# istellartech/OpenGoddard

Hardware: AMD Instinct MI355X
Metric: NLP-callback evals/sec (cost+constr+FD-Jacobian) (higher is better)
Workload: dtype f64; 1 GPU; polar_tsto: 2 phases, [6, 6] states, [3, 3] controls, [80, 80] LGL nodes; n=1442, m_eq=975, m_ineq=640, output_buffers=17 registered persistent-zero replicas of 18.6 MB in rotation, parallelism=fd-columns x1

## Files before the change

### __graft_entry__.py

```python
import os
import subprocess
import sys

ROOT = os.path.dirname(os.path.abspath(__file__))
if ROOT not in sys.path:
    sys.path.insert(0, ROOT)

PREBUILT = ("brachistochrone", "goddard", "polar_tsto_shipped", "polar_tsto",
            "low_thrust_shipped", "low_thrust", "launch4", "table_ascent", "low_thrust_r1", "launch4_r1",
            "goddard_1knot", "polar_ssto")


BEYOND_8192_NODES = [208, 208, 208, 208]
BOTH_CORES_NODES = [30]
NEAR_THE_LIMIT_NODES = [341, 341, 341, 341]


def build():
    from opengoddard_amd import build as ogbuild
    from opengoddard_amd import _native, codegen, problems
    print("[build] libogpsx.so ->", ogbuild.build_core(), flush=True)
    _native.lib()
    print("[build] libogsqp.so ->", ogbuild.build_sqp(), flush=True)
    from opengoddard_amd import _sqp_native
# ... 17 lines not shown
        import test_random_layouts
        extra = [factory() for factory in test_edge_problems.CASES.values()]
        extra += [test_random_layouts.make_problem(shape, seed) for seed, shape in test_random_layouts.CASES]
        for i, (prob, obj) in enumerate(extra):
            headers.append(("test problem %d" % i, codegen.emit_header(codegen.trace_problem(prob, obj))))
        import test_module_limits
        for key in test_module_limits.SHAPES:
            prob, obj = test_module_limits.problem(key)
            headers.append(("limit shape " + key, codegen.emit_header(codegen.trace_problem(prob, obj))))
            if key in test_module_limits.NOT_FITTING:
                batched.append(headers[-1])
        import test_fused_no_barrier
        for key in sorted(test_fused_no_barrier.SHAPES):
            prob, obj = test_fused_no_barrier.problem(key)
            headers.append(("no-barrier shape " + key, codegen.emit_header(codegen.trace_problem(prob, obj))))
        import test_exact_surface
        for name in test_exact_surface.BATCHED:
            prob, obj = test_exact_surface.build_problem(name)
            batched.append(("surface " + name, codegen.emit_header(codegen.trace_problem(prob, obj))))
        import warnings
        import parameter_cases
        for label, factory, with_batch in parameter_cases.modules():
            prob, obj = factory()
            with warnings.catch_warnings():
                warnings.simplefilter("ignore", RuntimeWarning)
                headers.append((label, codegen.emit_header(codegen.trace_problem(prob, obj))))
            if with_batch:
                batched.append(headers[-1])
                parametered.append(headers[-1])
        import og_math_cases
# ... 177 lines not shown
```

### opengoddard_amd/csrc/ogk.h

```cpp
#pragma once
#include <stdint.h>

#define OGK_ABI 14
#define OGK_MAX_PHASE 32

static inline int ogk_frag_nt(int N) { return (N + 15) / 16; }
static inline int ogk_frag_ks(int N) { return (N + 3) / 4; }
static inline long ogk_frag_size(int N) { return (long)ogk_frag_nt(N) * ogk_frag_ks(N) * 64; }
static inline void ogk_frag_pack(int N, const double* D, double* frag) {
    const int NT = ogk_frag_nt(N), KS = ogk_frag_ks(N);
    for (int nt = 0; nt < NT; ++nt)
        for (int ks = 0; ks < KS; ++ks)
            for (int lane = 0; lane < 64; ++lane) {
                const int k = 16 * nt + (lane & 15), l = 4 * ks + (lane >> 4);
                frag[((long)nt * KS + ks) * 64 + lane] = (k < N && l < N) ? D[(long)k * N + l] : 0.0;
            }
}

#define OGK_OTHER_PART (-4242)

enum ogk_mode {
    OGK_EVAL = 0,
    OGK_SWEEP = 1,
    OGK_DENSE = 2,
// ... 45 lines not shown
#define OGK_PART_HVP 9
#define OGK_PART_MIX 10
#define OGK_PART_HESS 11

enum ogk_flag {
    OGK_FLAG_COUNT_A = 0,
    OGK_FLAG_COUNT_B = 1,
    OGK_FLAG_TICKET = 2,
    OGK_FLAG_FUSED_COUNT = 3,
    OGK_FLAG_FUSED_RESULT = 4,
    OGK_FLAG_WORDS = 8
};

#ifdef __cplusplus
static_assert(OGK_FUSED == 5 && OGK_SWEEP == 1 && OGK_DENSE == 2, "og_sweep_mode's values are public (include/ogpsx.h)");
#endif

typedef struct ogk_info {
    int32_t abi;
    int32_t n, m, m_eq, m_ineq;
    int32_t n_phase, n_mv, n_groups, n_cvec;
    int32_t n_y0;
    int32_t phase_nodes[OGK_MAX_PHASE];
    int32_t n_eval_blocks;
    int32_t fused_ok;
} ogk_info;

typedef struct ogk_par_info {
    int32_t n_par, par_off;
} ogk_par_info;
// ... 5 lines not shown
    const double* cvec;
    double* f0;
    double* y0;
    double* xop;
    double* t0;
    double* z;
    int* nonfinite;
    int* nonfinite_next;
    unsigned* ready;
    double* jt;
    int32_t jt_sparse;
    int32_t jt_bump;
    uint32_t* jt_launches;
    uint32_t* jt_state;
    int* nonfinite_result;
    int32_t col_lo, col_hi;
    const int64_t* poff;
    const int64_t* pind;
    const int32_t* prow;
    int32_t* pint;
    double* pvals;
    double* ptail;
    int32_t ulo, uhi;
    double* trace;
    int64_t dfrag_off[OGK_MAX_PHASE];
} ogk_args;

#define OGK_BATCH_SETS 3
typedef struct ogk_batch_args {
    ogk_args* lanes;
// ... 22 lines not shown
```

### opengoddard_amd/csrc/ogk_fused_workgroup.inc

```
    int id = (int)blockIdx.x;
    if (id < n_eval) {
        FZ_TRACE_DECL(0);
        if (!(OGK_FZ & 16)) {
            if (id < ndef) eval_defect_body<true>(a, id, lds);
            else eval_rows_body<true>(a, id - ndef, lds);
        }
        FZ_STAMP(1);
        finish_eval(a, (unsigned)n_eval, reinterpret_cast<unsigned*>(lds));
        FZ_STAMP(4);
        FZ_TRACE_OUT(a);
        return;
    }
    id -= n_eval;
#ifndef OGK_ORDER
#define OGK_ORDER 0
#endif
    const int n_tile = OGT_N_FTILES, n_heavy = OGT_N_HPART;
    int kind, idx;
    if (OGK_ORDER == 0) {
        if (id < n_light) kind = 0, idx = id;
        else if (id < n_light + n_heavy) kind = 1, idx = id - n_light;
        else kind = 2, idx = id - n_light - n_heavy;
    } else if (OGK_ORDER == 1) {
        if (id < n_tile) kind = 2, idx = id;
        else if (id < n_tile + n_heavy) kind = 1, idx = id - n_tile;
        else kind = 0, idx = id - n_tile - n_heavy;
    } else {
        if (id < n_heavy) kind = 1, idx = id;
        else {
            const int r = id - n_heavy, pairs = n_light < n_tile ? n_light : n_tile;
            if (r < 2 * pairs) kind = (r & 1) ? 0 : 2, idx = r >> 1;
            else if (n_light > n_tile) kind = 0, idx = r - pairs;
            else kind = 2, idx = r - pairs;
        }
    }
    if (kind == 0)
        fz_light_body(a, n_sum < 0 ? group_lo + idx
                                   : idx < n_sum ? OGT_LSUM[sum_lo + idx] : OGT_LPLAIN[group_lo - sum_lo + idx - n_sum], lds);
    else if (kind == 1) { if (!(OGK_FZ & 32)) fz_heavy_part(a, idx, lds); }
    else fz_tile_body(a, idx, lds);
```

### opengoddard_amd/csrc/ogk_kernels.hip

```cpp
#include <hip/hip_runtime.h>
#include "ogk.h"
#include "og_dual.h"
#if defined(OGK_PART) && (OGK_PART == OGK_PART_HVP || OGK_PART == OGK_PART_MIX || OGK_PART == OGK_PART_HESS)
#include "og_dual2.h"
#endif
#include OG_GEN_HEADER

typedef double v4f64 __attribute__((ext_vector_type(4)));

#ifndef OGK_EXP
#define OGK_EXP 0
#endif

#ifndef OGK_TRACE
#define OGK_TRACE 0
#endif

namespace {

struct XCol {
    typedef double scalar;
    const double* x0;
    int j;
    double xj;
// ... 368 lines not shown
            const ogdual op = OgGen::mv_operand(si, l, xd, a.cvec);
            for (int k = tid; k < N; k += 256) {
                double v = __builtin_fma(op.d, dfrag_entry(a, phase, N, k, l), 0.0);
                if ((reads & 2) || ((reads & 1) && k == l)) v = v - OgGen::tail_one(si, k, xd, a.cvec).d;
                jrow[row0 + k] = v;
            }
        }
    }
}
#endif

constexpr int SWEEP_THREADS = 512;
constexpr int SWEEP_WAVES = SWEEP_THREADS / 64;

template <bool FUSED>
__device__ __forceinline__ void publish_row(const ogk_args& a, const int row, const double val) {
    const double zz = val - val;
    a.f0[row] = val;
    if (FUSED) __hip_atomic_store(&a.z[row], zz, __ATOMIC_RELAXED, __HIP_MEMORY_SCOPE_AGENT);
    else a.z[row] = zz;
    if (zz != zz) atomicAdd(a.nonfinite, 1);
}

template <bool FUSED>
__device__ __forceinline__ void eval_defect_body(const ogk_args& a, const int bx, double* lds) {
    const int4 blk = OGT_EVALBLK[bx];
    const int nt = blk.y, mv0 = blk.z, nmv = blk.w;
    const ogt_int8 rec0 = OGT_SLOT[mv0];
    const int N = rec0.v[0];
    const int KS = (N + 3) >> 2;
    const int NP = KS * 4;
    const int tid = (int)threadIdx.x;
    const int wave = tid >> 6, lane = tid & 63, lk = lane >> 4;

    double* dpanel = lds;
    double* xt = lds + KS * 64;
    double* ybuf = xt + OgGen::MAX_NMV * NP;
    const double* src = a.dfrag + a.dfrag_off[rec0.v[5]] + (long)nt * KS * 64;
    constexpr int UNR = 4;
// ... 52 lines not shown
    double T[TR];
#pragma unroll
    for (int r = 0; r < TR; ++r) {
        const int s = wave + r * SWEEP_WAVES;
        T[r] = (node_on && s < nmv) ? OgGen::tail_one(mv0 + s, k, base, a.cvec) : 0.0;
    }
    __syncthreads();
    if (!node_on) return;
#pragma unroll
    for (int r = 0; r < TR; ++r) {
        const int s = wave + r * SWEEP_WAVES;
        if (s >= nmv) break;
        const ogt_int8 rec = OGT_SLOT[mv0 + s];
        const double y = ybuf[s * 16 + lane];
        const int row = rec.v[3] + k;
        publish_row<FUSED>(a, row, y - T[r]);
        a.t0[row] = T[r];
        a.y0[rec.v[4] + k] = y;
    }
}

template <bool FUSED>
__device__ __forceinline__ void eval_rows_body(const ogk_args& a, const int bx, double* lds) {
    bool terms = false;
    if (TERM_CACHE) {
#pragma unroll
        for (int u = 0; u < SWEEP_WAVES; ++u) {
            const int w2 = bx * SWEEP_WAVES + u;
            if (w2 < OGT_N_ROWWAVES) terms = terms || OGT_ROWWAVE[w2].w != 0;
        }
        if (terms) {
            fill_terms<SWEEP_THREADS>(a, lds);
            __syncthreads();
        }
    }
    const int w = bx * SWEEP_WAVES + ((int)threadIdx.x >> 6);
    if (w >= OGT_N_ROWWAVES) return;
    const int4 rw = OGT_ROWWAVE[w];
    const int k = rw.y + ((int)threadIdx.x & 63);
    if (k >= rw.z) return;
    const XColT base = make_xcolt(a, -1, 0.0, terms ? lds : nullptr);
    int row;
    const double v = OgGen::item_value(rw.x, 0, k, base, a.y0, a.cvec, &row);
    publish_row<FUSED>(a, row, v);
}

#ifdef OGK_HAS_MAIN
__global__ __launch_bounds__(SWEEP_THREADS) void ogk_eval(const ogk_args a, const int ndef) {
    extern __shared__ __attribute__((aligned(16))) double lds[];
    const int id = (int)blockIdx.x;
    if (id == 0 && threadIdx.x == 0) {
        *a.nonfinite_next = 0;
        if (a.jt_bump) __hip_atomic_store(a.jt_launches, *a.jt_launches + 1u, __ATOMIC_RELAXED, __HIP_MEMORY_SCOPE_AGENT);
    }
    if (id < ndef) eval_defect_body<false>(a, id, lds);
    else eval_rows_body<false>(a, id - ndef, lds);
}
#endif

#ifndef OGK_LIGHT_COLS
#define OGK_LIGHT_COLS 4
#endif
constexpr int LIGHT_COLS = OGK_LIGHT_COLS;
constexpr int HEAVY_FLAG = 1 << 30;

__device__ __forceinline__ bool marked(const unsigned* bits, const int r) {
    return (bits[r >> 5] >> (r & 31)) & 1u;
}

__device__ __forceinline__ void fill_row(const ogk_args& a, double* jrow, const unsigned* bits,
                                         const int own_lo, const int own_hi, const int first,
// ... 254 lines not shown
    }
#endif
}

#ifndef OGK_FZ
#define OGK_FZ 0
#endif


__device__ __forceinline__ void lds_barrier() {
    __builtin_amdgcn_fence(__ATOMIC_RELEASE, "workgroup", "local");
    __builtin_amdgcn_s_barrier();
    __builtin_amdgcn_fence(__ATOMIC_ACQUIRE, "workgroup", "local");
}

__device__ __forceinline__ void fz_fill_from_z(const ogk_args& a, unsigned* bits) {
    const int tid = (int)threadIdx.x;
    for (int j = a.col_lo; j < a.col_hi; ++j) {
        const int4 col = OGT_COL[j];
        const int own_lo = col.z, own_hi = col.w & ~HEAVY_FLAG;
        for (int w = tid; w < ROW_WORDS; w += SWEEP_THREADS) bits[w] = 0u;
        __syncthreads();
        for (int e = col.x + tid; e < col.y; e += SWEEP_THREADS) {
            const int r = OGT_ELEM[e].w;
            atomicOr(&bits[r >> 5], 1u << (r & 31));
        }
        __syncthreads();
        fill_row(a, a.jt + (long)(j - a.col_lo) * OgGen::M, bits, own_lo, own_hi, tid, SWEEP_THREADS, false, true);
        __syncthreads();
    }
}

__device__ __forceinline__ void finish_eval(const ogk_args& a, const unsigned n_eval, unsigned* bits) {
    __shared__ int s_last;
    __builtin_amdgcn_s_waitcnt(0);
    __syncthreads();
    if (threadIdx.x == 0) {
        const unsigned t = __hip_atomic_fetch_add(a.ready, 1u, __ATOMIC_RELAXED, __HIP_MEMORY_SCOPE_AGENT);
        int last = 0;
        if (t + 1u == n_eval) {
            const int bad = __hip_atomic_load(a.nonfinite, __ATOMIC_RELAXED, __HIP_MEMORY_SCOPE_AGENT);
            const unsigned st = __hip_atomic_load(a.jt_state, __ATOMIC_RELAXED, __HIP_MEMORY_SCOPE_AGENT);
            const unsigned gen = __hip_atomic_load(a.jt_launches, __ATOMIC_RELAXED, __HIP_MEMORY_SCOPE_AGENT) + 1u;
            __hip_atomic_store(a.ready, 0u, __ATOMIC_RELAXED, __HIP_MEMORY_SCOPE_AGENT);
            __hip_atomic_store(a.jt_launches, gen, __ATOMIC_RELAXED, __HIP_MEMORY_SCOPE_AGENT);
            __hip_atomic_store(a.nonfinite_result, bad, __ATOMIC_RELAXED, __HIP_MEMORY_SCOPE_AGENT);
            if (a.ptail) a.ptail[OgGen::M] = (double)bad;
            __hip_atomic_store(a.nonfinite, 0, __ATOMIC_RELAXED, __HIP_MEMORY_SCOPE_AGENT);
            if (bad != 0) __hip_atomic_store(a.jt_state, gen, __ATOMIC_RELAXED, __HIP_MEMORY_SCOPE_AGENT);
            last = (bad != 0 || st == gen - 1u) ? 1 : 0;
        }
        s_last = last;
    }
    __syncthreads();
    if (s_last) fz_fill_from_z(a, bits);
}

template <int CH>
__device__ __forceinline__ void fz_load_panel(const double* bsrc, const int ks0, const int KS, double (&bv)[CH]) {
#pragma unroll
    for (int u = 0; u < CH; ++u) {
        const int ks = ks0 + u;
        const double v = bsrc[(ks < KS ? ks : KS - 1) * 64];
        bv[u] = ks < KS ? v : 0.0;
    }
}

template <int CH>
__device__ __forceinline__ void fz_load_first(const double* bsrc, const int KS, double (&b0)[CH], double (&b1)[CH]) {
    fz_load_panel<CH>(bsrc, 0, KS, b0);
// ... 281 lines not shown
            for (int r = 0; r < FZ_ROUNDS; ++r) {
                const double v = tyo[r] >= 0 ? t.yb[tyo[r] - y0_first] - tv[r] : tv[r];
                const double v0 = __shfl_down(v, 32);
                if (!base_role && il < cnt[r]) {
                    const double q = (v - v0) / dx;
                    jrow[trow[r]] = q;
                    if (pcol) pcol[tpos[r]] = q;
                }
            }
        }
    }
    FZ_STAMP(4);
    FZ_TRACE_OUT(a);
}

__device__ __forceinline__ void fz_tile_body(const ogk_args& a, const int bx, double* lds) {
    __shared__ int s_flags[4];
    FZ_TRACE_DECL(3);
    fz_sync_reset(s_flags, 4);
    const int4 tile = OGT_FTILE[bx];
    const int slot = tile.x, ct0 = tile.y, nt = tile.z, nct = tile.w;
    const ogt_int8 rec = OGT_SLOT[slot];
    const int N = rec.v[0], leaf = rec.v[2], row0 = rec.v[3];
    const bool diag = rec.v[6] & 1, generic = rec.v[6] & 2;
    const int dep0 = rec.v[7] >> 12, ndep = rec.v[7] & 0xfff;
    const int KS = (N + 3) >> 2;
    const int tid = (int)threadIdx.x;
    const int wave = tid >> 6, lane = tid & 63, lk = lane >> 4, kk = lane & 15;
    double* xt = lds;
    double* yb = lds + FZ_NP;
    double* tb = yb + 16;
// ... 37 lines not shown
        const XCol xa{a.x0, leaf + la, xa_b + xa_h};
        hit_v = OgGen::mv_operand(slot, la, xa, a.cvec);
    }
    if (col_on || wave == prod_wave) lds_count_wait(&s_flags[3], n_stage);
    FZ_STAMP(1);
    if (!col_wave) {
        if (wave == diag_wave) {
            if (diag_here && lk == 0 && k_on && leaf + k >= a.col_lo && leaf + k < a.col_hi) {
                const int jd = leaf + k;
                const double xbd = a.x0[jd];
                const XCol xd{a.x0, jd, xbd + a.h[jd]};
                td[kk] = OgGen::tail_one(slot, k, xd, a.cvec);
            }
            if (lane == 0) lds_count_up(&s_flags[2]);
        }
        if (wave == term_wave && lk == 0) tb[kk] = k_on ? OgGen::tail_one(slot, k, xbase, a.cvec) : 0.0;
        if (wave == term_wave && lane == 0) lds_count_up(&s_flags[1]);
        if (wave == prod_wave) {
            const v4f64 accb = fz_chain<CH>(bsrc, KS, b0, b1, [&](const int ks) {
                const double v = xt[(ks < KS ? ks : 0) * 4 + lk];
                return ks < KS ? v : 0.0;
            });
            if (lk == 0) yb[kk] = accb[0];
            FZ_STAMP(2);
            if (lane == 0) lds_count_up(&s_flags[0]);
        }
        FZ_TRACE_OUT(a);
        return;
    }
    if (!col_on) return;
    const int row = row0 + (k_on ? k : 0);
    double t_diag = 0.0;
    bool have_diag = false;
    {
        const int lc = k;
        const int reg = (lc - l0 - lk) >> 2;
        have_diag = diag && k_on && lc >= l0 + lk && ((lc - l0 - lk) & 3) == 0 && reg < 4 && lc < N &&
                    leaf + lc >= a.col_lo && leaf + lc < a.col_hi;
        if (have_diag && diag_wave < 0) {
            const int jd = leaf + lc;
// ... 39 lines not shown
            }
        }
        const double val = acc[reg] - t;
        const double q = (val - f_base) / dx;
        a.jt[(long)(j - a.col_lo) * OgGen::M + row] = q;
        if (a.pvals) a.pvals[a.poff[j] + k] = q;
    }
    FZ_STAMP(4);
    FZ_TRACE_OUT(a);
}

#ifndef OGK_FUSED_ATTR
#define OGK_FUSED_ATTR __attribute__((amdgpu_waves_per_eu(4)))
#endif
#ifdef OGK_HAS_FUSED
__global__ __launch_bounds__(SWEEP_THREADS) OGK_FUSED_ATTR void ogk_fused(const ogk_args a, const int ndef, const int n_eval,
                                                           const int group_lo, const int n_light, const int sum_lo,
                                                           const int n_sum) {
    extern __shared__ __attribute__((aligned(16))) double lds[];
#include "ogk_fused_workgroup.inc"
}
#endif

#if defined(OGK_HAS_BATCH) || defined(OGK_HAS_BATCH_EXACT) || defined(OGK_HAS_PAR) || defined(OGK_HAS_DIR) || \
    defined(OGK_HAS_ADJ) || defined(OGK_HAS_HVP) || defined(OGK_HAS_MIX) || defined(OGK_HAS_HESS)
typedef const ogk_args __attribute__((address_space(4))) * ogk_lane_table;
__device__ __forceinline__ const ogk_args& batch_lane(const ogk_args* lanes) {
    return *(const ogk_args*)((ogk_lane_table)lanes + blockIdx.y);
}
#endif

#ifdef OGK_HAS_BATCH
__global__ __launch_bounds__(SWEEP_THREADS) OGK_FUSED_ATTR void ogk_fused_batch(const ogk_args* __restrict__ lanes,
                                                                 const int ndef, const int n_eval, const int group_lo,
                                                                 const int n_light, const int sum_lo, const int n_sum) {
    extern __shared__ __attribute__((aligned(16))) double lds[];
    const ogk_args& a = batch_lane(lanes);
#include "ogk_fused_workgroup.inc"
}

__global__ __launch_bounds__(SWEEP_THREADS) void ogk_eval_batch(const ogk_args* __restrict__ lanes, const int ndef) {
    extern __shared__ __attribute__((aligned(16))) double lds[];
    const ogk_args& a = batch_lane(lanes);
    const int id = (int)blockIdx.x;
    if (id == 0 && threadIdx.x == 0) {
        *a.nonfinite_next = 0;
        if (a.jt_bump) __hip_atomic_store(a.jt_launches, *a.jt_launches + 1u, __ATOMIC_RELAXED, __HIP_MEMORY_SCOPE_AGENT);
    }
    if (id < ndef) eval_defect_body<false>(a, id, lds);
    else eval_rows_body<false>(a, id - ndef, lds);
}

__global__ void ogk_batch_bind(const ogk_batch_args b) {
    const int i = (int)(blockIdx.x * blockDim.x + threadIdx.x);
    if (i >= OGK_BATCH_SETS * b.capacity) return;
    const int k = i % b.capacity;
    ogk_args& a = b.lanes[i];
    a.x0 = b.X + (long)k * OgGen::N_VAR;
    a.h = b.H ? b.H + (long)k * OgGen::N_VAR : nullptr;
    a.f0 = b.F0 + (long)k * OgGen::M;
    a.pvals = b.vals ? b.vals + (long)k * b.nnz : nullptr;
    if (i / b.capacity == b.clear_set && k < b.count) *a.nonfinite = 0;
}
#endif

// ... 612 lines not shown
    return worst > terms ? worst : terms;
}

bool eval_lds_fits() { return defect_lds_bytes() <= 160 * 1024; }

size_t sweep_lds_bytes() { return (size_t)LIGHT_COLS * ROW_WORDS * sizeof(unsigned); }

int eval_row_blocks() { return (OGT_N_ROWWAVES + SWEEP_WAVES - 1) / SWEEP_WAVES; }

size_t fused_lds_bytes() {
    size_t bytes = defect_lds_bytes() > FZ_LDS_BYTES ? defect_lds_bytes() : FZ_LDS_BYTES;
    const size_t fill_lds = (size_t)ROW_WORDS * sizeof(unsigned);
    return fill_lds > bytes ? fill_lds : bytes;
}

bool fused_fits() { return fused_lds_bytes() <= 64 * 1024 && defect_blocks() + eval_row_blocks() > 0; }

int fused_light_order(long workgroups, int n_sum) { return workgroups <= 512 ? -1 : n_sum; }

}

namespace {
template <class G> constexpr auto gen_n_par(int) -> decltype(G::N_PAR) { return G::N_PAR; }
template <class G> constexpr int gen_n_par(long) { return 0; }
template <class G> constexpr auto gen_par_off(int) -> decltype(G::PAR_OFF) { return G::PAR_OFF; }
template <class G> constexpr int gen_par_off(long) { return G::N_CVEC; }
}

extern "C" int ogk_get_par_info(ogk_par_info* out) {
    out->n_par = gen_n_par<OgGen>(0);
    out->par_off = gen_par_off<OgGen>(0);
    return 0;
}

extern "C" int ogk_get_info(ogk_info* out) {
    out->abi = OGK_ABI;
    out->n_eval_blocks = defect_blocks() + eval_row_blocks();
    out->fused_ok = fused_fits() ? 1 : 0;
    out->n = OgGen::N_VAR;
    out->m = OgGen::M;
    out->m_eq = OgGen::M_EQ;
    out->m_ineq = OgGen::M_INEQ;
    out->n_phase = OgGen::N_PHASE;
    out->n_mv = OgGen::N_MV;
    out->n_groups = OgGen::N_GROUPS;
    out->n_cvec = OgGen::N_CVEC;
    out->n_y0 = OgGen::N_Y0;
    for (int i = 0; i < OGK_MAX_PHASE; ++i)
        out->phase_nodes[i] = i < OgGen::N_PHASE ? OgGen::PHASE_NODES(i) : 0;
    return 0;
}

// ... 42 lines not shown
        return (int)hipGetLastError();
    }
#endif
#ifdef OGK_HAS_FUSED
    if (mode == OGK_FUSED) {
        if (ncols <= 0) return 0;
        int glo = 0, ghi = OGT_N_LGRP;
        while (glo < ghi && OGH_LGRP_J[glo + 1] <= args->col_lo) ++glo;
        while (ghi > glo && OGH_LGRP_J[ghi - 1] >= args->col_hi) --ghi;
        if (!args->jt_sparse || !fused_fits()) return (int)hipErrorInvalidValue;
        int sum_lo = 0, n_sum = 0;
        for (int gidx = 0; gidx < ghi; ++gidx) {
            if (gidx < glo) sum_lo += OGH_LGRP_SUM[gidx];
            else n_sum += OGH_LGRP_SUM[gidx];
        }
        const int n_eval = ndef + eval_row_blocks();
        const int grid = n_eval + OGT_N_FTILES + OGT_N_HPART + (ghi - glo);
        hipLaunchKernelGGL(ogk_fused, dim3(grid), dim3(SWEEP_THREADS), fused_lds_bytes(), stream, *args, ndef, n_eval,
                           glo, ghi - glo, sum_lo, fused_light_order(grid, n_sum));
        return (int)hipGetLastError();
    }
#endif
#ifdef OGK_HAS_AUX
    if (mode == OGK_EXACT) {
        if (ncols <= 0) return 0;
        hipLaunchKernelGGL(ogk_exact_struct, dim3(ncols), dim3(256), 0, stream, *args);
        return (int)hipGetLastError();
    }
    if (mode == OGK_EXACT_DENSE) {
        if (ncols <= 0) return 0;
        int n_items = OgGen::N_ROW_ITEMS;
        for (int g = 0; g < OgGen::N_GROUPS; ++g)
            if (OgGen::G_KIND(g) == 1) n_items += OgGen::G_LEN(g);
// ... 84 lines not shown
        const int records = OGK_BATCH_SETS * b->capacity;
        hipLaunchKernelGGL(ogk_batch_bind, dim3((records + 63) / 64), dim3(64), 0, stream, *b);
        return (int)hipGetLastError();
    }
    if (mode == OGK_BATCH_EVAL) {
        if (!eval_lds_fits()) return (int)hipErrorInvalidValue;
        if (n_eval > 0)
            hipLaunchKernelGGL(ogk_eval_batch, dim3(n_eval, b->count), dim3(SWEEP_THREADS),
                               defect_lds_bytes(), stream, (const ogk_args*)b->lanes, ndef);
        return (int)hipGetLastError();
    }
    if (mode == OGK_BATCH_FUSED) {
        if (!fused_fits()) return (int)hipErrorInvalidValue;
        int n_sum = 0;
        for (int gidx = 0; gidx < OGT_N_LGRP; ++gidx) n_sum += OGH_LGRP_SUM[gidx];
        const int grid = n_eval + OGT_N_FTILES + OGT_N_HPART + OGT_N_LGRP;
        hipLaunchKernelGGL(ogk_fused_batch, dim3(grid, b->count), dim3(SWEEP_THREADS), fused_lds_bytes(), stream,
                           (const ogk_args*)b->lanes, ndef, n_eval, 0, OGT_N_LGRP, 0,
                           fused_light_order((long)grid * b->count, n_sum));
        return (int)hipGetLastError();
    }
    return (int)hipErrorInvalidValue;
}
#endif

#ifdef OGK_HAS_BATCH_EXACT
extern "C" int ogk_launch_batch(const ogk_batch_args* b, int mode, void* stream_) {
    hipStream_t stream = (hipStream_t)stream_;
    if (!b || !b->lanes || b->count < 1 || b->count > b->capacity || mode != OGK_BATCH_EXACT) return (int)hipErrorInvalidValue;
    const int grid = OgGen::N_HEAVY + (OgGen::N_VAR + XB_COLS - 1) / XB_COLS;
    hipLaunchKernelGGL(ogk_exact_struct_batch, dim3(grid, b->count), dim3(XB_THREADS), 0, stream,
                       (const ogk_args*)b->lanes);
    return (int)hipGetLastError();
// ... 110 lines not shown
```

### opengoddard_amd/csrc/ogpsx_core.hip

```cpp
#include <hip/hip_runtime.h>
#include <dlfcn.h>

#include <algorithm>
#include <chrono>
#include <cmath>
#include <cstdio>
#include <cstdlib>
#include <cstring>
#include <limits>
#include <mutex>
#include <string>
#include <vector>

#include "../../include/ogpsx.h"
#include "og_lgl.h"
#include "ogk.h"

namespace {

thread_local std::string g_error;

int fail(int code, const std::string& msg) {
    g_error = msg;
    return code;
// ... 62 lines not shown
    double* d_dfrag = nullptr;
    double* d_cvec = nullptr;
    int n_cvec = 0, n_par = 0, par_off = 0;
    double* d_theta = nullptr;
    int64_t dfrag_off[OGK_MAX_PHASE] = {0};
    double* d_x = nullptr;
    double* d_h = nullptr;
    double* d_f0 = nullptr;
    double* d_jt = nullptr;
    size_t jt_capacity = 0;
    double* d_y0 = nullptr;
    double* d_xop = nullptr;
    double* d_t0 = nullptr;
    double* d_z = nullptr;
    int* d_flags = nullptr;
    int flag_slot = 0;
    int n_eval_blocks = 0;
    double* d_trace = nullptr;
    int sweep_mode = OGK_FUSED;
    int exact_mode = OGK_EXACT;
    hipStream_t stream = nullptr;
    struct jt_reg {
        double* ptr;
        int lo, hi;
        int slot;
    };
    std::vector<jt_reg> regs;
    uint32_t* d_state = nullptr;
    bool fused_ok = false;
    int* nf_read = nullptr;
// ... 94 lines not shown
void fill_args(og_problem_s* p, ogk_args* a, const double* x, const double* h, double* f0,
               double* jt, int lo, int hi, bool new_launch = true) {
    memset(a, 0, sizeof *a);
    a->x0 = x;
    a->h = h;
    a->dfrag = p->d_dfrag;
    a->cvec = p->d_cvec;
    a->f0 = f0;
    a->y0 = p->d_y0;
    a->xop = p->d_xop;
    a->t0 = p->d_t0;
    a->z = p->d_z;
    a->nonfinite = p->d_flags + p->flag_slot;
    a->nonfinite_next = p->d_flags + (p->flag_slot ^ 1);
    a->ready = reinterpret_cast<unsigned*>(p->d_flags + OGK_FLAG_TICKET);
    a->trace = p->d_trace;
    a->jt = jt;
    a->col_lo = lo;
    a->col_hi = hi;
    a->jt_sparse = 0;
    a->jt_bump = 0;
    a->jt_state = p->d_state;
    a->jt_launches = p->d_state + 1;
    a->nonfinite_result = p->d_flags + OGK_FLAG_FUSED_RESULT;
    if (!new_launch && p->nf_read) a->nonfinite = p->nf_read;
    if (const og_problem_s::jt_reg* r = jt ? find_jt_reg(p, jt, lo, hi) : nullptr) {
        a->jt_sparse = 1;
        a->jt_state = p->d_state + 2 * r->slot;
        a->jt_launches = a->jt_state + 1;
    }
// ... 501 lines not shown
        e = hipMalloc(&p->d_cvec, sizeof(double) * (size_t)desc->n_cvec);
        if (e == hipSuccess)
            e = hipMemcpy(p->d_cvec, desc->cvec, sizeof(double) * (size_t)desc->n_cvec,
                          hipMemcpyHostToDevice);
    }
    if (e == hipSuccess && p->n_par > 0) e = hipMalloc(&p->d_theta, sizeof(double) * (size_t)p->n_par);
    if (e == hipSuccess) e = hipMalloc(&p->d_x, sizeof(double) * 2 * (size_t)p->n);
    if (e == hipSuccess) p->d_h = p->d_x + p->n;
    if (e == hipSuccess) e = hipMalloc(&p->d_f0, sizeof(double) * (size_t)p->m);
    if (e == hipSuccess) e = hipMalloc(&p->d_y0, sizeof(double) * (size_t)(info.n_y0 > 0 ? info.n_y0 : 1));
    if (e == hipSuccess) e = hipMalloc(&p->d_xop, sizeof(double) * (size_t)(info.n_y0 > 0 ? info.n_y0 : 1));
    if (e == hipSuccess) e = hipMalloc(&p->d_t0, sizeof(double) * (size_t)p->m);
    if (e == hipSuccess) e = hipMalloc(&p->d_z, sizeof(double) * (size_t)p->m);
    if (e == hipSuccess) e = hipMalloc(&p->d_flags, OGK_FLAG_WORDS * sizeof(int));
    if (e == hipSuccess) e = hipMemset(p->d_flags, 0, OGK_FLAG_WORDS * sizeof(int));
    if (e == hipSuccess && getenv("OGPSX_TRACE")) {
        e = hipMalloc(&p->d_trace, sizeof(double) * OG_TRACE_DOUBLES);
        if (e == hipSuccess) e = hipMemset(p->d_trace, 0, sizeof(double) * OG_TRACE_DOUBLES);
    }
    if (e == hipSuccess) e = hipMalloc(&p->d_state, 2 * (OG_MAX_JT_REGS + 2) * sizeof(uint32_t));
    if (e == hipSuccess) e = hipMemset(p->d_state, 0xff, 2 * (OG_MAX_JT_REGS + 2) * sizeof(uint32_t));
    if (e == hipSuccess) e = hipMemset(p->d_state + 2 * (OG_MAX_JT_REGS + 1) + 1, 0, sizeof(uint32_t));
    p->n_eval_blocks = info.n_eval_blocks;
    p->fused_ok = info.fused_ok != 0;
    const char* mode_env = getenv("OGPSX_SWEEP");
    p->sweep_mode = OGK_FUSED;
    if (mode_env && std::string(mode_env) == "dense") p->sweep_mode = OGK_DENSE, p->exact_mode = OGK_EXACT_DENSE;
    if (mode_env && std::string(mode_env) == "split") p->sweep_mode = OGK_SWEEP;
    if (mode_env && std::string(mode_env) == "fused") p->sweep_mode = OGK_FUSED;
    if (p->n_eval_blocks <= 0 && p->sweep_mode == OGK_FUSED) p->sweep_mode = OGK_SWEEP;
// ... 26 lines not shown
    hipFree(p->d_pj);
    hipFree(p->d_dir);
    hipFree(p->d_adj);
    hipFree(p->d_hvp);
    hipFree(p->d_mix);
    hipFree(p->d_hess_plan);
    hipFree(p->d_hess);
    hipFree(p->d_x);
    hipFree(p->d_f0);
    hipFree(p->d_jt);
    hipFree(p->d_y0);
    hipFree(p->d_xop);
    hipFree(p->d_t0);
    hipFree(p->d_z);
    hipFree(p->d_flags);
    hipFree(p->d_state);
    hipFree(p->d_trace);
    hipFree(p->d_indptr);
    hipFree(p->d_rows);
    hipFree(p->d_down);
    hipFree(p->d_shard_off);
    for (auto& r : p->host_regs)
        if (r.mapped && r.registered_here) (void)hipHostUnregister(r.ptr);
    (void)hipGetLastError();
    if (p->h_up) hipHostFree(p->h_up);
    if (p->h_xh) hipHostFree(p->h_xh);
    if (p->h_down) hipHostFree(p->h_down);
    for (hipEvent_t ev : p->down_ev)
        if (ev) hipEventDestroy(ev);
    for (int k = 1; k < p->launch.n_parts; ++k)
// ... 444 lines not shown
    return download_block(p, lo, hi, JT, F0);
}

}

struct og_batch_s {
    og_problem_s* p = nullptr;
    int capacity = 0;
    int64_t nnz = 0;
    ogk_args* d_table = nullptr;
    std::vector<ogk_args> table;
    double* d_jt = nullptr;
    double* d_scratch = nullptr;
    size_t scratch_lane = 0, n_y0 = 0;
    int* d_flags = nullptr;
    uint32_t* d_state = nullptr;
    std::vector<int> nf_word;
    hipStream_t last_stream = nullptr;
    double *d_xh = nullptr, *d_f = nullptr, *d_vals = nullptr;
    double *h_up = nullptr, *h_down = nullptr;
    int* h_flags = nullptr;
    double* d_cvec = nullptr;
    double *d_th = nullptr, *h_th = nullptr;
    double* d_pj = nullptr;
    double* d_dj = nullptr;
    double* d_aj = nullptr;
    double* d_hj = nullptr;
    double* d_mj = nullptr;
    double* d_hm = nullptr;
};
// ... 135 lines not shown

void og_batch_destroy(og_batch b) {
    if (!b || !live_batch(b)) return;
    {
        std::lock_guard<std::mutex> guard(g_batches_lock);
        g_batches.erase(std::find(g_batches.begin(), g_batches.end(), b));
    }
    og_problem_s* p = b->p;
    auto it = std::find(p->batches.begin(), p->batches.end(), b);
    if (it != p->batches.end()) p->batches.erase(it);
    hipSetDevice(p->device);
    hipFree(b->d_table);
    hipFree(b->d_jt);
    hipFree(b->d_scratch);
    hipFree(b->d_flags);
    hipFree(b->d_state);
    hipFree(b->d_xh);
    hipFree(b->d_f);
    hipFree(b->d_vals);
    hipFree(b->d_cvec);
    hipFree(b->d_th);
    hipFree(b->d_pj);
    hipFree(b->d_dj);
    hipFree(b->d_aj);
    hipFree(b->d_hj);
    hipFree(b->d_mj);
    hipFree(b->d_hm);
    if (b->h_th) hipHostFree(b->h_th);
    if (b->h_up) hipHostFree(b->h_up);
    if (b->h_down) hipHostFree(b->h_down);
// ... 23 lines not shown
    b->nnz = p->indptr[(size_t)p->n];
    b->n_y0 = (size_t)(info.n_y0 > 0 ? info.n_y0 : 1);
    b->scratch_lane = 2 * b->n_y0 + 2 * (size_t)p->m;
    b->nf_word.assign((size_t)capacity, OGK_FLAG_FUSED_RESULT);
    {
        std::lock_guard<std::mutex> guard(g_batches_lock);
        g_batches.push_back(b);
    }
    p->batches.push_back(b);
    const size_t cap = (size_t)capacity, n = (size_t)p->n, m = (size_t)p->m, nnz = (size_t)(b->nnz ? b->nnz : 1);
    hipError_t e = hipMalloc(&b->d_jt, sizeof(double) * cap * n * m);
    if (e == hipSuccess) e = hipMemsetAsync(b->d_jt, 0, sizeof(double) * cap * n * m, p->stream);
    if (e == hipSuccess) e = hipMalloc(&b->d_scratch, sizeof(double) * cap * b->scratch_lane);
    if (e == hipSuccess) e = hipMalloc(&b->d_flags, sizeof(int) * OGK_FLAG_WORDS * cap);
    if (e == hipSuccess) e = hipMemsetAsync(b->d_flags, 0, sizeof(int) * OGK_FLAG_WORDS * cap, p->stream);
    if (e == hipSuccess) e = hipMalloc(&b->d_state, sizeof(uint32_t) * 2 * cap);
    if (e == hipSuccess) e = hipMalloc(&b->d_table, sizeof(ogk_args) * OGK_BATCH_SETS * cap);
    if (e == hipSuccess) e = hipMalloc(&b->d_xh, sizeof(double) * 2 * cap * n);
    if (e == hipSuccess) e = hipMalloc(&b->d_f, sizeof(double) * cap * m);
    if (e == hipSuccess) e = hipMalloc(&b->d_vals, sizeof(double) * cap * nnz);
    if (e == hipSuccess) e = hipHostMalloc(&b->h_up, sizeof(double) * 2 * cap * n, hipHostMallocDefault);
    if (e == hipSuccess) e = hipHostMalloc(&b->h_down, sizeof(double) * cap * (nnz + m), hipHostMallocDefault);
    if (e == hipSuccess) e = hipHostMalloc(&b->h_flags, sizeof(int) * OGK_FLAG_WORDS * cap, hipHostMallocDefault);
    if (p->n_par > 0) {
        const size_t nc = (size_t)p->n_cvec, np_ = (size_t)p->n_par;
        if (e == hipSuccess) e = hipMalloc(&b->d_cvec, sizeof(double) * cap * nc);
        for (size_t k = 0; e == hipSuccess && k < cap; ++k)
            e = hipMemcpyAsync(b->d_cvec + k * nc, p->d_cvec, sizeof(double) * nc, hipMemcpyDeviceToDevice, p->stream);
        if (e == hipSuccess) e = hipMalloc(&b->d_th, sizeof(double) * cap * np_);
        if (e == hipSuccess) e = hipHostMalloc(&b->h_th, sizeof(double) * cap * np_, hipHostMallocDefault);
// ... 10 lines not shown
                ogk_args& a = b->table[(size_t)set * cap + k];
                fill_args(p, &a, nullptr, nullptr, nullptr, nullptr, 0, p->n);
                double* scr = b->d_scratch + k * b->scratch_lane;
                int* fl = b->d_flags + OGK_FLAG_WORDS * k;
                a.y0 = scr;
                a.xop = scr + b->n_y0;
                a.t0 = scr + 2 * b->n_y0;
                a.z = a.t0 + m;
                a.trace = nullptr;
                if (b->d_cvec) a.cvec = b->d_cvec + k * (size_t)p->n_cvec;
                a.jt = b->d_jt + k * n * m;
                a.jt_sparse = 1;
                a.jt_state = b->d_state + 2 * k;
                a.jt_launches = a.jt_state + 1;
                a.ready = reinterpret_cast<unsigned*>(fl + OGK_FLAG_TICKET);
                a.nonfinite_result = fl + OGK_FLAG_FUSED_RESULT;
                a.poff = p->d_indptr;
                if (set == 0) {
                    a.nonfinite = fl + OGK_FLAG_FUSED_COUNT;
                    a.nonfinite_next = fl + OGK_FLAG_FUSED_COUNT;
                } else {
                    a.nonfinite = fl + OGK_FLAG_COUNT_A;
                    a.nonfinite_next = fl + OGK_FLAG_COUNT_B;
                    a.jt_bump = set - 1;
                }
            }
        e = hipMemcpy(b->d_table, b->table.data(), sizeof(ogk_args) * b->table.size(), hipMemcpyHostToDevice);
    }
    if (e == hipSuccess) e = hipStreamSynchronize(p->stream);
    if (e != hipSuccess) {
// ... 1410 lines not shown
```

Measured before the change: 691.7 million callback evals/s.

## Publish defect rows from fused tiles and use packed 64-bit ticket/count completion

New measurement: 690.9 million callback evals/s. No clear change (-0.1%).

```diff
diff --git a/__graft_entry__.py b/__graft_entry__.py
--- a/__graft_entry__.py
+++ b/__graft_entry__.py
@@ -55,6 +55,13 @@
         for key in sorted(test_fused_no_barrier.SHAPES):
             prob, obj = test_fused_no_barrier.problem(key)
             headers.append(("no-barrier shape " + key, codegen.emit_header(codegen.trace_problem(prob, obj))))
+        import test_fused_publish
+        for key in sorted(test_fused_publish.SHAPES):
+            prob, obj = test_fused_publish.problem(key)
+            header = codegen.emit_header(codegen.trace_problem(prob, obj))
+            if header not in set(h for _, h in headers):
+                headers.append(("publish shape " + key, header))
+            batched.append(("publish shape " + key, header))
         import test_exact_surface
         for name in test_exact_surface.BATCHED:
             prob, obj = test_exact_surface.build_problem(name)
diff --git a/opengoddard_amd/csrc/ogk.h b/opengoddard_amd/csrc/ogk.h
--- a/opengoddard_amd/csrc/ogk.h
+++ b/opengoddard_amd/csrc/ogk.h
@@ -1,7 +1,7 @@
 #pragma once
 #include <stdint.h>
 
-#define OGK_ABI 14
+#define OGK_ABI 15
 #define OGK_MAX_PHASE 32
 
 static inline int ogk_frag_nt(int N) { return (N + 15) / 16; }
@@ -83,6 +83,7 @@
 
 #ifdef __cplusplus
 static_assert(OGK_FUSED == 5 && OGK_SWEEP == 1 && OGK_DENSE == 2, "og_sweep_mode's values are public (include/ogpsx.h)");
+static_assert(OGK_FLAG_TICKET % 2 == 0 && OGK_FLAG_FUSED_COUNT == OGK_FLAG_TICKET + 1, "one 64-bit word: ticket | count");
 #endif
 
 typedef struct ogk_info {
@@ -118,6 +119,7 @@
     uint32_t* jt_launches;
     uint32_t* jt_state;
     int* nonfinite_result;
+    uint32_t* nanmap;
     int32_t col_lo, col_hi;
     const int64_t* poff;
     const int64_t* pind;
diff --git a/opengoddard_amd/csrc/ogk_fused_workgroup.inc b/opengoddard_amd/csrc/ogk_fused_workgroup.inc
--- a/opengoddard_amd/csrc/ogk_fused_workgroup.inc
+++ b/opengoddard_amd/csrc/ogk_fused_workgroup.inc
@@ -1,12 +1,12 @@
     int id = (int)blockIdx.x;
     if (id < n_eval) {
         FZ_TRACE_DECL(0);
-        if (!(OGK_FZ & 16)) {
-            if (id < ndef) eval_defect_body<true>(a, id, lds);
-            else eval_rows_body<true>(a, id - ndef, lds);
-        }
+        FzHistory hst = {0u, 0u};
+        if (threadIdx.x < 64) hst = fz_history(a);
+        bool bad = false;
+        if (!(OGK_FZ & 16)) bad = eval_rows_body<true>(a, id, lds);
         FZ_STAMP(1);
-        finish_eval(a, (unsigned)n_eval, reinterpret_cast<unsigned*>(lds));
+        finish_rows(a, (unsigned)n_part, bad, hst);
         FZ_STAMP(4);
         FZ_TRACE_OUT(a);
         return;
@@ -38,4 +38,4 @@
         fz_light_body(a, n_sum < 0 ? group_lo + idx
                                    : idx < n_sum ? OGT_LSUM[sum_lo + idx] : OGT_LPLAIN[group_lo - sum_lo + idx - n_sum], lds);
     else if (kind == 1) { if (!(OGK_FZ & 32)) fz_heavy_part(a, idx, lds); }
-    else fz_tile_body(a, idx, lds);
+    else fz_tile_body(a, idx, (unsigned)n_part, lds);
diff --git a/opengoddard_amd/csrc/ogk_kernels.hip b/opengoddard_amd/csrc/ogk_kernels.hip
--- a/opengoddard_amd/csrc/ogk_kernels.hip
+++ b/opengoddard_amd/csrc/ogk_kernels.hip
@@ -406,15 +406,21 @@
 constexpr int SWEEP_WAVES = SWEEP_THREADS / 64;
 
 template <bool FUSED>
-__device__ __forceinline__ void publish_row(const ogk_args& a, const int row, const double val) {
+__device__ __forceinline__ bool publish_row(const ogk_args& a, const int row, const double val) {
     const double zz = val - val;
     a.f0[row] = val;
-    if (FUSED) __hip_atomic_store(&a.z[row], zz, __ATOMIC_RELAXED, __HIP_MEMORY_SCOPE_AGENT);
-    else a.z[row] = zz;
-    if (zz != zz) atomicAdd(a.nonfinite, 1);
-}
-
-template <bool FUSED>
+    a.z[row] = zz;
+    const bool bad = zz != zz;
+    if (!FUSED && bad) atomicAdd(a.nonfinite, 1);
+    return bad;
+}
+
+__device__ __forceinline__ void fz_mark_nan(const ogk_args& a, const int row) {
+    const unsigned old = __hip_atomic_fetch_or(&a.nanmap[row >> 5], 1u << (row & 31), __ATOMIC_RELAXED,
+                                               __HIP_MEMORY_SCOPE_AGENT);
+    asm volatile("s_waitcnt vmcnt(0)" : : "v"(old) : "memory");
+}
+
 __device__ __forceinline__ void eval_defect_body(const ogk_args& a, const int bx, double* lds) {
     const int4 blk = OGT_EVALBLK[bx];
     const int nt = blk.y, mv0 = blk.z, nmv = blk.w;
@@ -497,14 +503,14 @@
         const ogt_int8 rec = OGT_SLOT[mv0 + s];
         const double y = ybuf[s * 16 + lane];
         const int row = rec.v[3] + k;
-        publish_row<FUSED>(a, row, y - T[r]);
+        publish_row<false>(a, row, y - T[r]);
         a.t0[row] = T[r];
         a.y0[rec.v[4] + k] = y;
     }
 }
 
 template <bool FUSED>
-__device__ __forceinline__ void eval_rows_body(const ogk_args& a, const int bx, double* lds) {
+__device__ __forceinline__ bool eval_rows_body(const ogk_args& a, const int bx, double* lds) {
     bool terms = false;
     if (TERM_CACHE) {
 #pragma unroll
@@ -518,14 +524,16 @@
         }
     }
     const int w = bx * SWEEP_WAVES + ((int)threadIdx.x >> 6);
-    if (w >= OGT_N_ROWWAVES) return;
+    if (w >= OGT_N_ROWWAVES) return false;
     const int4 rw = OGT_ROWWAVE[w];
     const int k = rw.y + ((int)threadIdx.x & 63);
-    if (k >= rw.z) return;
+    if (k >= rw.z) return false;
     const XColT base = make_xcolt(a, -1, 0.0, terms ? lds : nullptr);
     int row;
     const double v = OgGen::item_value(rw.x, 0, k, base, a.y0, a.cvec, &row);
-    publish_row<FUSED>(a, row, v);
+    const bool bad = publish_row<FUSED>(a, row, v);
+    if (FUSED && bad) fz_mark_nan(a, row);
+    return bad;
 }
 
 #ifdef OGK_HAS_MAIN
@@ -536,8 +544,8 @@
         *a.nonfinite_next = 0;
         if (a.jt_bump) __hip_atomic_store(a.jt_launches, *a.jt_launches + 1u, __ATOMIC_RELAXED, __HIP_MEMORY_SCOPE_AGENT);
     }
-    if (id < ndef) eval_defect_body<false>(a, id, lds);
-    else eval_rows_body<false>(a, id - ndef, lds);
+    if (id < ndef) eval_defect_body(a, id, lds);
+    else (void)eval_rows_body<false>(a, id - ndef, lds);
 }
 #endif
 
@@ -822,46 +830,76 @@
     __builtin_amdgcn_fence(__ATOMIC_ACQUIRE, "workgroup", "local");
 }
 
-__device__ __forceinline__ void fz_fill_from_z(const ogk_args& a, unsigned* bits) {
-    const int tid = (int)threadIdx.x;
+
+struct FzHistory { unsigned st, gen0; };
+__device__ __forceinline__ FzHistory fz_history(const ogk_args& a) {
+    FzHistory hst;
+    hst.st = __hip_atomic_load(a.jt_state, __ATOMIC_RELAXED, __HIP_MEMORY_SCOPE_AGENT);
+    hst.gen0 = __hip_atomic_load(a.jt_launches, __ATOMIC_RELAXED, __HIP_MEMORY_SCOPE_AGENT);
+    return hst;
+}
+
+__device__ __forceinline__ void fz_fill_wave(const ogk_args& a, const bool nan_rows) {
+    const int lane = (int)threadIdx.x & 63, bit = lane & 31;
     for (int j = a.col_lo; j < a.col_hi; ++j) {
         const int4 col = OGT_COL[j];
         const int own_lo = col.z, own_hi = col.w & ~HEAVY_FLAG;
-        for (int w = tid; w < ROW_WORDS; w += SWEEP_THREADS) bits[w] = 0u;
-        __syncthreads();
-        for (int e = col.x + tid; e < col.y; e += SWEEP_THREADS) {
-            const int r = OGT_ELEM[e].w;
-            atomicOr(&bits[r >> 5], 1u << (r & 31));
-        }
-        __syncthreads();
-        fill_row(a, a.jt + (long)(j - a.col_lo) * OgGen::M, bits, own_lo, own_hi, tid, SWEEP_THREADS, false, true);
-        __syncthreads();
-    }
-}
-
-__device__ __forceinline__ void finish_eval(const ogk_args& a, const unsigned n_eval, unsigned* bits) {
-    __shared__ int s_last;
-    __builtin_amdgcn_s_waitcnt(0);
-    __syncthreads();
-    if (threadIdx.x == 0) {
-        const unsigned t = __hip_atomic_fetch_add(a.ready, 1u, __ATOMIC_RELAXED, __HIP_MEMORY_SCOPE_AGENT);
-        int last = 0;
-        if (t + 1u == n_eval) {
-            const int bad = __hip_atomic_load(a.nonfinite, __ATOMIC_RELAXED, __HIP_MEMORY_SCOPE_AGENT);
-            const unsigned st = __hip_atomic_load(a.jt_state, __ATOMIC_RELAXED, __HIP_MEMORY_SCOPE_AGENT);
-            const unsigned gen = __hip_atomic_load(a.jt_launches, __ATOMIC_RELAXED, __HIP_MEMORY_SCOPE_AGENT) + 1u;
-            __hip_atomic_store(a.ready, 0u, __ATOMIC_RELAXED, __HIP_MEMORY_SCOPE_AGENT);
-            __hip_atomic_store(a.jt_launches, gen, __ATOMIC_RELAXED, __HIP_MEMORY_SCOPE_AGENT);
-            __hip_atomic_store(a.nonfinite_result, bad, __ATOMIC_RELAXED, __HIP_MEMORY_SCOPE_AGENT);
-            if (a.ptail) a.ptail[OgGen::M] = (double)bad;
-            __hip_atomic_store(a.nonfinite, 0, __ATOMIC_RELAXED, __HIP_MEMORY_SCOPE_AGENT);
-            if (bad != 0) __hip_atomic_store(a.jt_state, gen, __ATOMIC_RELAXED, __HIP_MEMORY_SCOPE_AGENT);
-            last = (bad != 0 || st == gen - 1u) ? 1 : 0;
-        }
-        s_last = last;
-    }
-    __syncthreads();
-    if (s_last) fz_fill_from_z(a, bits);
+        double* jrow = a.jt + (long)(j - a.col_lo) * OgGen::M;
+        for (int c = 0; c < ROW_WORDS; c += 64) {
+            const int w = c + lane;
+            unsigned written = 0u, nanw = 0u;
+            for (int e = col.x; e < col.y; ++e) {
+                const int r = OGT_ELEM[e].w;
+                if ((r >> 5) == w) written |= 1u << (r & 31);
+            }
+            if (nan_rows && w < ROW_WORDS) nanw = __hip_atomic_load(&a.nanmap[w], __ATOMIC_RELAXED, __HIP_MEMORY_SCOPE_AGENT);
+#pragma unroll 1
+            for (int i = 0; i < 32; ++i) {
+                const int src = 2 * i + (lane >> 5);
+                const unsigned wr = __shfl(written, src), nn = __shfl(nanw, src);
+                const int r = (c + src) * 32 + bit;
+                if (r < OgGen::M && (r < own_lo || r >= own_hi) && !((wr >> bit) & 1u))
+                    jrow[r] = ((nn >> bit) & 1u) ? __builtin_nan("") : 0.0;
+            }
+        }
+    }
+    if (nan_rows)
+        for (int w = lane; w < ROW_WORDS; w += 64)
+            __hip_atomic_store(&a.nanmap[w], 0u, __ATOMIC_RELAXED, __HIP_MEMORY_SCOPE_AGENT);
+}
+
+__device__ __forceinline__ void fz_finish(const ogk_args& a, const unsigned n_part, const int bad_own, const FzHistory hst) {
+    const int lane = (int)threadIdx.x & 63;
+    unsigned long long t = 0ull;
+    if (lane == 0)
+        t = __hip_atomic_fetch_add(reinterpret_cast<unsigned long long*>(a.ready),
+                                   1ull | ((unsigned long long)(unsigned)bad_own << 32), __ATOMIC_RELAXED,
+                                   __HIP_MEMORY_SCOPE_AGENT);
+    const unsigned before = __builtin_amdgcn_readfirstlane((unsigned)t);
+    if (before + 1u != n_part) return;
+    const int bad = (int)__builtin_amdgcn_readfirstlane((unsigned)(t >> 32)) + bad_own;
+    const unsigned st = __builtin_amdgcn_readfirstlane(hst.st), gen = __builtin_amdgcn_readfirstlane(hst.gen0) + 1u;
+    if (lane == 0) {
+        __hip_atomic_store(reinterpret_cast<unsigned long long*>(a.ready), 0ull, __ATOMIC_RELAXED, __HIP_MEMORY_SCOPE_AGENT);
+        __hip_atomic_store(a.jt_launches, gen, __ATOMIC_RELAXED, __HIP_MEMORY_SCOPE_AGENT);
+        __hip_atomic_store(a.nonfinite_result, bad, __ATOMIC_RELAXED, __HIP_MEMORY_SCOPE_AGENT);
+        if (a.ptail) a.ptail[OgGen::M] = (double)bad;
+        if (bad != 0) __hip_atomic_store(a.jt_state, gen, __ATOMIC_RELAXED, __HIP_MEMORY_SCOPE_AGENT);
+    }
+    if (bad != 0 || st == gen - 1u) fz_fill_wave(a, bad != 0);
+}
+
+__device__ __forceinline__ void finish_rows(const ogk_args& a, const unsigned n_part, const bool bad_lane, const FzHistory hst) {
+    __shared__ int s_bad[SWEEP_WAVES];
+    const int wave = (int)threadIdx.x >> 6, lane = (int)threadIdx.x & 63;
+    const int mine = __popcll(__ballot(bad_lane));
+    if (lane == 0) s_bad[wave] = mine;
+    lds_barrier();
+    if (wave != 0) return;
+    int bad = 0;
+#pragma unroll
+    for (int u = 0; u < SWEEP_WAVES; ++u) bad += s_bad[u];
+    fz_finish(a, n_part, bad, hst);
 }
 
 template <int CH>
@@ -1173,7 +1211,7 @@
     FZ_TRACE_OUT(a);
 }
 
-__device__ __forceinline__ void fz_tile_body(const ogk_args& a, const int bx, double* lds) {
+__device__ __forceinline__ void fz_tile_body(const ogk_args& a, const int bx, const unsigned n_part, double* lds) {
     __shared__ int s_flags[4];
     FZ_TRACE_DECL(3);
     fz_sync_reset(s_flags, 4);
@@ -1241,7 +1279,11 @@
             }
             if (lane == 0) lds_count_up(&s_flags[2]);
         }
-        if (wave == term_wave && lk == 0) tb[kk] = k_on ? OgGen::tail_one(slot, k, xbase, a.cvec) : 0.0;
+        double t_own = 0.0;
+        if (wave == term_wave && lk == 0) {
+            t_own = k_on ? OgGen::tail_one(slot, k, xbase, a.cvec) : 0.0;
+            tb[kk] = t_own;
+        }
         if (wave == term_wave && lane == 0) lds_count_up(&s_flags[1]);
         if (wave == prod_wave) {
             const v4f64 accb = fz_chain<CH>(bsrc, KS, b0, b1, [&](const int ks) {
@@ -1251,6 +1293,17 @@
             if (lk == 0) yb[kk] = accb[0];
             FZ_STAMP(2);
             if (lane == 0) lds_count_up(&s_flags[0]);
+        }
+        if (wave == term_wave && ct0 == 0) {
+            if (term_wave != prod_wave) lds_count_wait(&s_flags[0], 1);
+            const FzHistory hst = fz_history(a);
+            bool bad = false;
+            if (lk == 0 && k_on) {
+                bad = publish_row<true>(a, row0 + k, yb[kk] - t_own);
+                if (bad) fz_mark_nan(a, row0 + k);
+            }
+            FZ_STAMP(3);
+            fz_finish(a, n_part, __popcll(__ballot(bad)), hst);
         }
         FZ_TRACE_OUT(a);
         return;
@@ -1320,7 +1373,7 @@
 #define OGK_FUSED_ATTR __attribute__((amdgpu_waves_per_eu(4)))
 #endif
 #ifdef OGK_HAS_FUSED
-__global__ __launch_bounds__(SWEEP_THREADS) OGK_FUSED_ATTR void ogk_fused(const ogk_args a, const int ndef, const int n_eval,
+__global__ __launch_bounds__(SWEEP_THREADS) OGK_FUSED_ATTR void ogk_fused(const ogk_args a, const int n_part, const int n_eval,
                                                            const int group_lo, const int n_light, const int sum_lo,
                                                            const int n_sum) {
     extern __shared__ __attribute__((aligned(16))) double lds[];
@@ -1338,7 +1391,7 @@
 
 #ifdef OGK_HAS_BATCH
 __global__ __launch_bounds__(SWEEP_THREADS) OGK_FUSED_ATTR void ogk_fused_batch(const ogk_args* __restrict__ lanes,
-                                                                 const int ndef, const int n_eval, const int group_lo,
+                                                                 const int n_part, const int n_eval, const int group_lo,
                                                                  const int n_light, const int sum_lo, const int n_sum) {
     extern __shared__ __attribute__((aligned(16))) double lds[];
     const ogk_args& a = batch_lane(lanes);
@@ -1353,8 +1406,8 @@
         *a.nonfinite_next = 0;
         if (a.jt_bump) __hip_atomic_store(a.jt_launches, *a.jt_launches + 1u, __ATOMIC_RELAXED, __HIP_MEMORY_SCOPE_AGENT);
     }
-    if (id < ndef) eval_defect_body<false>(a, id, lds);
-    else eval_rows_body<false>(a, id - ndef, lds);
+    if (id < ndef) eval_defect_body(a, id, lds);
+    else (void)eval_rows_body<false>(a, id - ndef, lds);
 }
 
 __global__ void ogk_batch_bind(const ogk_batch_args b) {
@@ -1997,7 +2050,15 @@
     return fill_lds > bytes ? fill_lds : bytes;
 }
 
-bool fused_fits() { return fused_lds_bytes() <= 64 * 1024 && defect_blocks() + eval_row_blocks() > 0; }
+int fused_publishers() {
+    int np = 0;
+    for (int g = 0; g < OgGen::N_GROUPS; ++g)
+        if (OgGen::G_KIND(g) == 1) np += OgGen::G_NMV(g) * ((OgGen::G_LEN(g) + 15) >> 4);
+    return np;
+}
+int fused_participants() { return eval_row_blocks() + fused_publishers(); }
+
+bool fused_fits() { return fused_lds_bytes() <= 64 * 1024 && fused_participants() > 0; }
 
 int fused_light_order(long workgroups, int n_sum) { return workgroups <= 512 ? -1 : n_sum; }
 
@@ -2018,7 +2079,7 @@
 
 extern "C" int ogk_get_info(ogk_info* out) {
     out->abi = OGK_ABI;
-    out->n_eval_blocks = defect_blocks() + eval_row_blocks();
+    out->n_eval_blocks = fused_participants();
     out->fused_ok = fused_fits() ? 1 : 0;
     out->n = OgGen::N_VAR;
     out->m = OgGen::M;
@@ -2091,9 +2152,10 @@
             if (gidx < glo) sum_lo += OGH_LGRP_SUM[gidx];
             else n_sum += OGH_LGRP_SUM[gidx];
         }
-        const int n_eval = ndef + eval_row_blocks();
+        const int n_eval = eval_row_blocks();
         const int grid = n_eval + OGT_N_FTILES + OGT_N_HPART + (ghi - glo);
-        hipLaunchKernelGGL(ogk_fused, dim3(grid), dim3(SWEEP_THREADS), fused_lds_bytes(), stream, *args, ndef, n_eval,
+        hipLaunchKernelGGL(ogk_fused, dim3(grid), dim3(SWEEP_THREADS), fused_lds_bytes(), stream, *args,
+                           fused_participants(), n_eval,
                            glo, ghi - glo, sum_lo, fused_light_order(grid, n_sum));
         return (int)hipGetLastError();
     }
@@ -2208,9 +2270,10 @@
         if (!fused_fits()) return (int)hipErrorInvalidValue;
         int n_sum = 0;
         for (int gidx = 0; gidx < OGT_N_LGRP; ++gidx) n_sum += OGH_LGRP_SUM[gidx];
-        const int grid = n_eval + OGT_N_FTILES + OGT_N_HPART + OGT_N_LGRP;
+        const int n_rows = eval_row_blocks();
+        const int grid = n_rows + OGT_N_FTILES + OGT_N_HPART + OGT_N_LGRP;
         hipLaunchKernelGGL(ogk_fused_batch, dim3(grid, b->count), dim3(SWEEP_THREADS), fused_lds_bytes(), stream,
-                           (const ogk_args*)b->lanes, ndef, n_eval, 0, OGT_N_LGRP, 0,
+                           (const ogk_args*)b->lanes, fused_participants(), n_rows, 0, OGT_N_LGRP, 0,
                            fused_light_order((long)grid * b->count, n_sum));
         return (int)hipGetLastError();
     }
diff --git a/opengoddard_amd/csrc/ogpsx_core.hip b/opengoddard_amd/csrc/ogpsx_core.hip
--- a/opengoddard_amd/csrc/ogpsx_core.hip
+++ b/opengoddard_amd/csrc/ogpsx_core.hip
@@ -100,6 +100,7 @@
     double* d_t0 = nullptr;
     double* d_z = nullptr;
     int* d_flags = nullptr;
+    uint32_t* d_nanmap = nullptr;
     int flag_slot = 0;
     int n_eval_blocks = 0;
     double* d_trace = nullptr;
@@ -224,6 +225,7 @@
     a->nonfinite = p->d_flags + p->flag_slot;
     a->nonfinite_next = p->d_flags + (p->flag_slot ^ 1);
     a->ready = reinterpret_cast<unsigned*>(p->d_flags + OGK_FLAG_TICKET);
+    a->nanmap = p->d_nanmap;
     a->trace = p->d_trace;
     a->jt = jt;
     a->col_lo = lo;
@@ -755,6 +757,8 @@
     if (e == hipSuccess) e = hipMalloc(&p->d_z, sizeof(double) * (size_t)p->m);
     if (e == hipSuccess) e = hipMalloc(&p->d_flags, OGK_FLAG_WORDS * sizeof(int));
     if (e == hipSuccess) e = hipMemset(p->d_flags, 0, OGK_FLAG_WORDS * sizeof(int));
+    if (e == hipSuccess) e = hipMalloc(&p->d_nanmap, sizeof(uint32_t) * (((size_t)p->m + 31) / 32));
+    if (e == hipSuccess) e = hipMemset(p->d_nanmap, 0, sizeof(uint32_t) * (((size_t)p->m + 31) / 32));
     if (e == hipSuccess && getenv("OGPSX_TRACE")) {
         e = hipMalloc(&p->d_trace, sizeof(double) * OG_TRACE_DOUBLES);
         if (e == hipSuccess) e = hipMemset(p->d_trace, 0, sizeof(double) * OG_TRACE_DOUBLES);
@@ -811,6 +815,7 @@
     hipFree(p->d_t0);
     hipFree(p->d_z);
     hipFree(p->d_flags);
+    hipFree(p->d_nanmap);
     hipFree(p->d_state);
     hipFree(p->d_trace);
     hipFree(p->d_indptr);
@@ -1285,6 +1290,7 @@
     double* d_scratch = nullptr;
     size_t scratch_lane = 0, n_y0 = 0;
     int* d_flags = nullptr;
+    uint32_t* d_nanmap = nullptr;
     uint32_t* d_state = nullptr;
     std::vector<int> nf_word;
     hipStream_t last_stream = nullptr;
@@ -1450,6 +1456,7 @@
     hipFree(b->d_jt);
     hipFree(b->d_scratch);
     hipFree(b->d_flags);
+    hipFree(b->d_nanmap);
     hipFree(b->d_state);
     hipFree(b->d_xh);
     hipFree(b->d_f);
@@ -1503,6 +1510,9 @@
     if (e == hipSuccess) e = hipMalloc(&b->d_scratch, sizeof(double) * cap * b->scratch_lane);
     if (e == hipSuccess) e = hipMalloc(&b->d_flags, sizeof(int) * OGK_FLAG_WORDS * cap);
     if (e == hipSuccess) e = hipMemsetAsync(b->d_flags, 0, sizeof(int) * OGK_FLAG_WORDS * cap, p->stream);
+    const size_t map_words = (m + 31) / 32;
+    if (e == hipSuccess) e = hipMalloc(&b->d_nanmap, sizeof(uint32_t) * map_words * cap);
+    if (e == hipSuccess) e = hipMemsetAsync(b->d_nanmap, 0, sizeof(uint32_t) * map_words * cap, p->stream);
     if (e == hipSuccess) e = hipMalloc(&b->d_state, sizeof(uint32_t) * 2 * cap);
     if (e == hipSuccess) e = hipMalloc(&b->d_table, sizeof(ogk_args) * OGK_BATCH_SETS * cap);
     if (e == hipSuccess) e = hipMalloc(&b->d_xh, sizeof(double) * 2 * cap * n);
@@ -1543,6 +1553,7 @@
                 a.jt_state = b->d_state + 2 * k;
                 a.jt_launches = a.jt_state + 1;
                 a.ready = reinterpret_cast<unsigned*>(fl + OGK_FLAG_TICKET);
+                a.nanmap = b->d_nanmap + k * map_words;
                 a.nonfinite_result = fl + OGK_FLAG_FUSED_RESULT;
                 a.poff = p->d_indptr;
                 if (set == 0) {
```
